# ksadov/FREUD

Hardware: AMD Instinct MI355X
Metric: SAE train activations/sec (d=384 dict 8x) (higher is better)
Workload: dtype bf16; 1 GPU; Whisper-tiny d=384 dict 8x (n=3072) L1 SAE train step, M=65536 rows/GPU/step, RAdam+cosine, x bfloat16 resident in HBM (BASELINE configs[1]); rows_per_gpu=65536, d_model=384, n_dict=3072, parallelism=dp1, dp=none

## Files before the change

### freud_amd/csrc/engine.hip

```cpp
#include <hip/hip_runtime.h>
#include <math.h>
#include <stdarg.h>
#include <stdio.h>
#include <string.h>

#include <algorithm>
#include <utility>
#include <vector>

#include "../../include/freud_sae.h"
#include "l1_kernels.h"
#include "gemm256.h"
#include "gemm256s.h"
#include "gemm256_fp8.h"
#include "l1_fp8.h"
#include "dp_kernels.h"
#include "p2p_exchange.h"
#include <rccl/rccl.h>
#include <mutex>
#include <unistd.h>

static thread_local bool g_force_gemm128 = false;
static thread_local bool g_no_stream = false;
static thread_local int g_device = 0;
// ... 115 lines not shown
  unsigned char *x8 = nullptr, *c8 = nullptr, *W8 = nullptr, *W8t = nullptr;
  float *scal8 = nullptr, *x8_part = nullptr;
  bool use_fused_fwd = false;
  int fwd_variant = 2;
  bf16_t *xb = nullptr, *c = nullptr, *dxh = nullptr, *dpre = nullptr;
  bf16_t *dxhT = nullptr, *xT = nullptr;
  float *slab = nullptr, *db_part = nullptr, *l1_part = nullptr, *sq_part = nullptr, *scal = nullptr;
  double* gn_part = nullptr;
  float* cn_part = nullptr;
  bool cn_valid = false;
  bool wb_valid = false;
  float* cnorm = nullptr;
  bool wn_pending = false, wn_fwd_seen = false;
  sae_grad_ready_fn grad_ready = nullptr;
  void* grad_ready_user = nullptr;
  int dw_chunk_rows = 0;
  int dw_chunk_splits = 1;
  int dw_col_chunks = 1;
  int dw_col_splits = 1;
  float* cnt_part = nullptr;
  int gn_blocks = 0;
  bool step_fused_call = false;
  bool gn_valid = false;
  bool metrics_fresh = false;
  const bf16_t* xb_cur = nullptr;
  unsigned int* masked = nullptr;
  int dw_splits = 1;
  int dw_tail_tiles = 0, dw_tail_pieces = 0;
  float* dw_tail = nullptr;
  int bwd_splits = 1;
  int bwd_range_splits = 1;
  bool use_fused_bwd = false;
  bool topk = false;
  int k = 0, k_aux_cap = 0;
  int64_t rows_per_file = 0;
  double dead_threshold = 1e300;
  bf16_t *We_b = nullptr, *Wd_b = nullptr, *xs = nullptr, *pre = nullptr, *dense = nullptr, *aux_dense = nullptr;
  bf16_t *de_b = nullptr, *dh_b = nullptr;
  float *e = nullptr, *dh = nullptr, *e2_part = nullptr, *a2_part = nullptr, *dbd_part = nullptr, *ds_part = nullptr, *tkf = nullptr;
  int *top_idx = nullptr, *aux_idx = nullptr, *tk = nullptr;
  bf16_t *top_vals = nullptr, *aux_vals = nullptr, *multi_vals = nullptr;
  unsigned short* tile_max = nullptr;
  unsigned char* sel_flag = nullptr;
  bool dense_valid = false;
  bool multi_dense_valid = false;
  float* be_r = nullptr;
// ... 289 lines not shown
  return SAE_OK;
}

extern "C" void sae_destroy(sae_ctx* c) {
  if (!c) return;
  (void)hipSetDevice(c->cfg.device_id);
  void* ptrs[] = {c->P,    c->Mom,     c->Var,     c->G,       c->Wb,   c->Wt,      c->xb,    c->c, c->dxh, c->dxhT, c->xT,
                  c->dpre, c->slab,    c->db_part, c->l1_part, c->sq_part, c->scal, c->gn_part, c->masked, c->cn_part, c->cnt_part,
                  c->We_b, c->Wd_b, c->xs, c->pre, c->dense, c->aux_dense, c->de_b, c->dh_b, c->e, c->dh, c->e2_part,
                  c->a2_part, c->dbd_part, c->ds_part, c->tkf, c->top_idx, c->aux_idx, c->tk, c->tv_part, c->nfsf, c->dead, c->dbe_fx,
                  c->multi_dense, c->multi_idx, c->em, c->dm_b, c->m2_part, c->x8, c->c8, c->W8, c->W8t, c->scal8, c->x8_part, c->dxh8,
                  c->stats, c->stats_part, c->Gb, c->top_vals, c->aux_vals, c->multi_vals, c->tile_max, c->sel_flag, c->csc_counts, c->csc_block_off, c->csc_total, c->csc_start, c->csc_item_start,
                  c->csc_item_latent, c->csc_entries, c->csc_part, c->csc_pbe, c->tkd, c->dead_cols, c->vec_rank, c->vec_bits, c->Wdd_b,
                  c->aux_dbe_part, c->be_r, c->cnorm, c->dw_tail, c->csc_multi, c->fs_slab};
  for (void* p : ptrs)
    if (p) (void)hipFree(p);
  if (c->dead_hint) (void)hipHostFree(c->dead_hint);
  for (int i = 0; i < c->p2p_nopened; ++i) (void)hipIpcCloseMemHandle(c->p2p_opened[i]);
  if (c->sig) (void)hipFree(c->sig);
  if (c->p2p_status) (void)hipFree(c->p2p_status);
  if (c->p2p_status_host) (void)hipHostFree(c->p2p_status_host);
  if (c->col_stage) (void)hipFree(c->col_stage);
  if (c->bal_map) (void)hipFree(c->bal_map);
  for (void* p : {(void*)c->e32_x, (void*)c->e32_pre, (void*)c->e32_sel, (void*)c->e32_xhat, (void*)c->e32_part, (void*)c->e32_colmax})
    if (p) (void)hipFree(p);
  if (c->comm) (void)ncclCommDestroy(c->comm);
  if (c->comm_stream) (void)hipStreamDestroy(c->comm_stream);
  for (hipEvent_t e : {c->ev_x, c->ev_stats, c->ev_done})
    if (e) (void)hipEventDestroy(e);
  for (hipEvent_t e : c->ev_range)
    if (e) (void)hipEventDestroy(e);
  if (c->ev_init)
    for (auto& r : c->ev)
      for (int i = 0; i < EV_RING; ++i) {
        if (r.beg[i]) (void)hipEventDestroy(r.beg[i]);
        if (r.end[i]) (void)hipEventDestroy(r.end[i]);
      }
  delete c;
}

extern "C" int sae_create(const sae_config* cfg, sae_ctx** out) {
  if (!cfg || !out) return fail(SAE_ERR_INVALID, "null argument");
  *out = nullptr;
  if (cfg->variant != SAE_VARIANT_L1 && cfg->variant != SAE_VARIANT_TOPK)
    return fail(SAE_ERR_INVALID, "Invalid autoencoder variant: %d, must be 'l1' or 'topk'", cfg->variant);
  if (cfg->variant == SAE_VARIANT_TOPK && (cfg->k <= 0 || cfg->k > cfg->n_dict || cfg->k > 1024))
// ... 159 lines not shown
  ALLOC(c->cnorm, (int64_t)c->n_p * 4);
  if (c->dw_tail_tiles > 0 || (c->d_p >= 1024 && c->d_p % 256 == 0 && c->n_p % 256 == 0)) ALLOC(c->dw_tail, (int64_t)256 * 65536 * 4);
  ALLOC(c->masked, 2048 * 4);
  ALLOC(c->cnt_part, (Mp / 128 + 1) * 4);
  c->stats_cap = DP_STATS_HEAD;
  if (!c->stats) ALLOC(c->stats, c->stats_cap * 8);
  ALLOC(c->stats_part, 1024 * 4);
  if (c->fp8) {
    ALLOC(c->x8, Mp * c->d_p);
    ALLOC(c->c8, Mp * c->n_p);
    ALLOC(c->W8, c->nW);
    ALLOC(c->W8t, c->nW);
    ALLOC(c->scal8, S8_COUNT * 4);
    ALLOC(c->x8_part, 2 * 1024 * 4);
    if (c->fp8_bwd) ALLOC(c->dxh8, Mp * c->d_p);
  }
#undef ALLOC
  {
    int rc_init = [&]() -> int {
      HIP_TRY(hipMemset(c->P, 0, c->nparams * 4));
      HIP_TRY(hipMemset(c->Mom, 0, c->nparams * 4));
      HIP_TRY(hipMemset(c->Var, 0, c->nparams * 4));
      HIP_TRY(hipMemset(c->G, 0, (c->nparams + SAE_NUM_METRICS) * 4));
      int rc_ev = create_events(c);
      if (rc_ev) return rc_ev;
      HIP_TRY(hipDeviceSynchronize());
      return SAE_OK;
    }();
    if (rc_init) {
      sae_destroy(c);
      return rc_init;
    }
  }
  *out = c;
  return SAE_OK;
}

static int copy2d(void* dst, size_t dpitch, const void* src, size_t spitch, size_t width, size_t height, int to_internal,
                  int is_device) {
  hipMemcpyKind kind = is_device ? hipMemcpyDeviceToDevice : (to_internal ? hipMemcpyHostToDevice : hipMemcpyDeviceToHost);
  HIP_TRY(hipMemcpy2D(dst, dpitch, src, spitch, width, height, kind));
  return SAE_OK;
}

static int xfer_flat(sae_ctx* c, float* internal, float* w_ext, float* b_ext, int to_internal, int is_device) {
  int rc;
// ... 910 lines not shown
    return SAE_OK;
  }
  rc = launch_encoder<T>(c, enc_gemm_args(c, c->xb_cur, Mp), M, s);
  if (rc) return rc;
  {
    GemmArgs g{};
    g.A0 = c->c; g.B0 = c->Wb; g.lda = n_p; g.ldb = n_p;
    g.nbm = (int)(Mp / 128); g.nbn = d_p / 128; g.ktiles0 = g.ktiles = n_p / 64; g.splits = 1;
    g.group_m = 4;
    EpiDec<T> e{};
    e.x = x; e.dxh = c->dxh; e.scal = c->scal; e.sq_part = c->sq_part; e.M = M; e.d = d; e.d_p = d_p; e.nbn = g.nbn;
    e.vec_all = (M == Mp && d == d_p && d % 4 == 0 && (reinterpret_cast<uintptr_t>(x) % (4 * sizeof(T))) == 0) ? 1 : 0;
    ev_begin(c, KID_DEC_FWD, s);
    rc = launch_gemm<OP_ROW, OP_ROW>(g, e, s);
    ev_end(c, KID_DEC_FWD, s);
    if (rc) return rc;
  }
  if (need_backward && c->dxhT) {
    hipLaunchKernelGGL(transpose_bf16_kernel, dim3((unsigned)(Mp / 64), d_p / 64), dim3(256), 0, s, c->dxh, c->dxhT, Mp, d_p);
    hipLaunchKernelGGL(transpose_bf16_kernel, dim3((unsigned)(Mp / 64), d_p / 64), dim3(256), 0, s, c->xb_cur, c->xT, Mp, d_p);
    HIP_TRY(hipGetLastError());
  }
  return SAE_OK;
}

template <typename T>
static int fwd_bwd_impl(sae_ctx* c, const T* x, int64_t M, hipStream_t s, bool backward) {
  const int d = c->d, d_p = c->d_p, n_p = c->n_p;
  const int64_t Mp = round_up(M, c->row_pad);
  const float alpha = (float)c->cfg.recon_alpha;
  const double* gs = (backward && c->dp_world > 0) ? c->stats : nullptr;
  ev_begin(c, KID_STEP_TOTAL, s);
  int rc = forward_impl<T>(c, x, M, Mp, s, backward);
  if (rc) return rc;
  const bool fold_finalize = c->use_fused_fwd && c->use_fused_bwd && backward && gs == nullptr && c->bwd_ranges == 1 &&
                             c->cfg.debug_flags != 78;
  if (c->use_fused_fwd && !fold_finalize) {
    StatsPush push{};
    if (gs && inline_stats(c)) {
      for (int r = 0; r < c->dp_world; ++r) push.inbox[r] = c->p2p_sig[r] + P2P_SIG_WORDS;
      push.rank = c->p2p_rank; push.world = c->dp_world; push.epoch = ++c->p2p_epoch_push;
      push.timeout_ticks = c->p2p_timeout_ticks; push.status = c->p2p_status; push.status_host = c->p2p_status_hostdev; push.gstats_out = c->stats;
    } else if (gs && c->dist) {
      HIP_TRY(hipStreamWaitEvent(s, c->ev_stats, 0));
    }
    if (push.world > 0) ev_begin(c, KID_STATS_XCHG, s);
// ... 161 lines not shown
        rc = launch_dw(g, e, r0);
        if (rc) return rc;
        if (direct && g.tail_tiles > 0)
          hipLaunchKernelGGL(reduce_tail_kernel, dim3(g.tail_tiles, 16), dim3(256), 0, s, c->dw_tail, c->G, n_p, d_p / 256, n_p / 256,
                             g.tail_tiles, g.tail_pieces);
        if (chunked) {
          const int64_t off4 = (int64_t)r0 * n_p / 4, n4 = (int64_t)rows * n_p / 4;
          hipLaunchKernelGGL(reduce_slabs_kernel, dim3((unsigned)((n4 + 255) / 256)), dim3(256), 0, s, c->slab + 4 * off4,
                             c->G + 4 * off4, n4, c->nW / 4, splits);
          notify_grads(c, 4 * off4, 4 * n4, s);
        }
      }
      if (!col_chunked) {
        ev_end(c, KID_DW, s);
        dw_chunked_any = chunked;
        dw_chunked = chunked || direct;
      }
    }
    ev_begin(c, KID_REDUCE, s);
    if (c->use_fused_bwd && c->bwd_ranges > 1) {
      c->gn_blocks = 256 * c->bwd_ranges;
      c->gn_valid = true;
    } else if (c->use_fused_bwd) {
      const int64_t nW4 = c->nW / 4, n4 = c->nparams / 4;
      const int blocks = grid_for(n4, 1024);
      LossFinalize fin{};
      if (fold_finalize) {
        fin.l1_part = c->l1_part; fin.sq_part = c->sq_part; fin.cnt_part = c->cnt_part; fin.n_parts = (int)(Mp / 128);
        fin.scal = c->scal; fin.metrics = c->G + c->nparams; fin.M = M; fin.d = d; fin.alpha = alpha;
      }
      hipLaunchKernelGGL(reduce_grads_kernel, dim3(blocks), dim3(256), 0, s, c->slab, nW4, splits, c->db_part, db_rows, n_p,
                         c->G, nW4, n4, c->gn_part,
                         (c->dist && c->dp_world > 0 && c->payload == SAE_DTYPE_BF16) ? c->Gb : (bf16_t*)nullptr, fin,
                         (c->bwd_ranges == 1 && c->bal_m > 0 && (int)(Mp / BF_BM) >= 64) ? c->bal_m : 0);
      c->gn_blocks = blocks;
      c->gn_valid = true;
    } else {
      const int64_t n4 = c->nW / 4;
      if (!dw_chunked)
        hipLaunchKernelGGL(reduce_slabs_kernel, dim3((unsigned)((n4 + 255) / 256)), dim3(256), 0, s, c->slab, c->G, n4, n4,
                           splits);
      hipLaunchKernelGGL(reduce_db_kernel, dim3(n_p / 32), dim3(256), 0, s, c->db_part, c->G + c->nW, db_rows, n_p);
      c->gn_valid = false;
    }
    ev_end(c, KID_REDUCE, s);
  }
  if (!c->use_fused_fwd)
    hipLaunchKernelGGL(finalize_losses_kernel, dim3(1), dim3(1024), 0, s, c->l1_part, (int)((Mp / 128) * (n_p / 128)),
                       c->sq_part, (int)((Mp / 128) * (d_p / 128)), c->scal, c->G + c->nparams, M, d, alpha,
                       (const float*)nullptr, 0, gs, StatsPush{});
  if (backward) {
    const int64_t total = c->nparams + SAE_NUM_METRICS;
    if (c->use_fused_bwd && c->dist && c->dp_world > 0) {
      const int nr = c->bwd_ranges, cols = n_p / nr;
      fused_exchange(c, nr - 1, nr, (nr - 1) * cols, cols, true, s);
    } else if (dw_chunked_any) notify_grads(c, c->nW, total - c->nW, s);
    else notify_grads(c, 0, total, s);
  }
  ev_end(c, KID_STEP_TOTAL, s);
// ... 544 lines not shown
  a.grad_scale = (float)grad_scale;
  a.clip_thresh = (float)c->cfg.clip_thresh;
  a.weight_decay = (float)c->cfg.weight_decay;
  a.beta1 = (float)b1;
  a.beta2 = (float)b2;
  a.eps = (float)c->cfg.eps;
  a.one_minus_beta1 = (float)(1.0 - b1);
  a.one_minus_beta2 = (float)(1.0 - b2);
  a.bc1 = (float)bc1;
  a.bc2_sqrt = (float)sqrt(bc2);
  a.step_size = (float)(lr / bc1);
  a.is_radam = c->cfg.optimizer == SAE_OPT_RADAM;
  a.scale_metrics = c->metrics_fresh ? 1 : 0;
  c->metrics_fresh = false;
  if (a.is_radam) {
    const double rho_inf = 2.0 / (1.0 - b2) - 1.0;
    const double rho_t = rho_inf - 2.0 * t * pow(b2, t) / bc2;
    a.rectify = rho_t > 5.0;
    a.rect = a.rectify ? (float)sqrt((rho_t - 4) * (rho_t - 2) * rho_inf / ((rho_inf - 4) * (rho_inf - 2) * rho_t)) : 0.f;
  }
  ev_begin(c, KID_OPT, s);
  const int64_t n4 = c->nparams / 4;
  int gblocks = grid_for(n4, 1024);
  if (c->grads_in_bf16) {
    hipLaunchKernelGGL(gnorm_from_bf16_kernel, dim3(gblocks), dim3(256), 0, s, c->Gb, c->G, n4, a.grad_scale, c->gn_part);
    c->grads_in_bf16 = false;
  } else if (c->gn_valid && grad_scale == 1.0 && c->step_fused_call) {
    gblocks = c->gn_blocks;
  } else {
    hipLaunchKernelGGL(gnorm_partial_kernel, dim3(gblocks), dim3(256), 0, s, c->G, n4, a.grad_scale, c->gn_part);
  }
  c->gn_valid = false;
  const int oblocks = grid_for(n4, 2048);
  if (!c->topk && !c->fp8 && c->d_p <= 384 && c->cfg.debug_flags != 79 && c->cfg.debug_flags != 80) {
    const int norm_on_load = (c->wn_pending && c->wn_fwd_seen) ? 1 : 0;
    hipLaunchKernelGGL(optimizer_l1_cols_kernel, dim3(c->n_p / OPTC_COLS + c->n_p / 128), dim3(OPTC_THREADS), optc_lds_bytes(c->d_p), s, c->P,
                       c->Mom, c->Var, c->G, c->d_p, c->n_p, c->gn_part, gblocks, a, c->G + c->nparams, c->cnorm, norm_on_load, c->Wb,
                       c->Wt);
    c->wn_pending = true;
    c->wn_fwd_seen = false;
    c->cn_valid = false;
  } else if (!c->topk && c->cfg.debug_flags != 79) {
    settle_weights(c, s);
    hipLaunchKernelGGL(optimizer_l1_kernel, dim3(c->n_p / 128, c->d_p / 32 + 1), dim3(256), 0, s, c->P, c->Mom, c->Var, c->G, c->d_p,
                       c->n_p, c->gn_part, gblocks, a, c->G + c->nparams, c->cn_part);
    c->cn_valid = true;
// ... 7 lines not shown
    hipLaunchKernelGGL(optimizer_kernel, dim3(oblocks), dim3(256), 0, s, c->P, c->Mom, c->Var, c->G, n4, c->gn_part, gblocks,
                       a, c->G + c->nparams, cast);
    c->cn_valid = false;
    c->wb_valid = c->topk;
  }
  if (c->topk)
    hipLaunchKernelGGL(nfsf_update_kernel, dim3((c->n + 255) / 256), dim3(256), 0, s, c->nfsf, c->G + c->nparams + SAE_NUM_METRICS,
                       c->n, (long long)(c->last_M * (grad_scale > 0 ? (long long)llround(1.0 / grad_scale) : 1)),
                       c->dp_world > 0 ? c->stats : (const double*)nullptr);
  ev_end(c, KID_OPT, s);
  HIP_TRY(hipGetLastError());
  return SAE_OK;
}

extern "C" int sae_set_topk_options(sae_ctx* c, double dead_feature_threshold, int64_t rows_per_file) {
  if (!c) return fail(SAE_ERR_INVALID, "null argument");
  if (!c->topk) return fail(SAE_ERR_STATE, "not a topk context");
  c->dead_threshold = dead_feature_threshold;
  c->rows_per_file = rows_per_file;
  return SAE_OK;
}

extern "C" int sae_step(sae_ctx* c, const void* x, int64_t M, int x_dtype, double lr, void* stream) {
  int rc = sae_forward_backward(c, x, M, x_dtype, stream);
  if (rc) return rc;
  c->step_fused_call = c->dp_world == 0 || c->gn_from_exchange;
  rc = sae_optimizer_step(c, lr, 1.0, stream);
  c->step_fused_call = false;
  return rc;
}

extern "C" int sae_read_metrics(sae_ctx* c, float out[SAE_NUM_METRICS], void* stream) {
  if (!c || !out) return fail(SAE_ERR_INVALID, "null argument");
  if (int rc = no_forward_left(c)) return rc;
  USE_DEVICE(c);
  HIP_TRY(hipMemcpyAsync(out, c->G + c->nparams, SAE_NUM_METRICS * 4, hipMemcpyDeviceToHost, (hipStream_t)stream));
  HIP_TRY(hipStreamSynchronize((hipStream_t)stream));
  return SAE_OK;
}

static int ensure_dense(sae_ctx* c) {
  if (!c->topk || c->dense_valid || c->last_M <= 0) return SAE_OK;
  HIP_TRY(hipDeviceSynchronize());
  hipLaunchKernelGGL(topk_densify_kernel, dim3((unsigned)c->last_M_p), dim3(256), 0, (hipStream_t)0, c->top_vals, c->top_idx, c->k,
                     c->dense, c->n_p);
  HIP_TRY(hipGetLastError());
  HIP_TRY(hipDeviceSynchronize());
  c->dense_valid = true;
  return SAE_OK;
}

extern "C" int sae_debug_read(sae_ctx* c, int which, float* out, int64_t cap) {
  if (!c || !out) return fail(SAE_ERR_INVALID, "null argument");
  USE_DEVICE(c);
  HIP_TRY(hipDeviceSynchronize());
  if (which == 0) {
    int rc_d = ensure_dense(c);
    if (rc_d) return rc_d;
  }
  const int64_t M = c->last_M;
// ... 54 lines not shown
  if (which == 12) {
    const int64_t rows = cap / 8 < 4096 ? cap / 8 : 4096;
    std::vector<unsigned long long> tmp((size_t)rows * 8);
    HIP_TRY(hipMemcpyFromSymbol(tmp.data(), HIP_SYMBOL(tsel_stamp_buf), tmp.size() * 8, 0, hipMemcpyDeviceToHost));
    for (int64_t i = 0; i < rows * 8; ++i) out[i] = (float)tmp[(size_t)i];
    return SAE_OK;
  }
#endif
  if (which == 11) {
    if (!c->topk || !c->aux_dense) return fail(SAE_ERR_INVALID, "no AuxK buffers");
    const int64_t rows = cap / 8 < c->last_M ? cap / 8 : c->last_M;
    std::vector<unsigned long long> tmp((size_t)rows * 8);
    HIP_TRY(hipMemcpy2D(tmp.data(), 64, reinterpret_cast<const char*>(c->aux_dense) + (size_t)c->n_p * 2 - 64, (size_t)c->n_p * 2, 64, (size_t)rows,
                        hipMemcpyDeviceToHost));
    for (int64_t i = 0; i < rows * 8; ++i) out[i] = (float)tmp[(size_t)i];
    return SAE_OK;
  }
  if (which == 5) {
    const int64_t nq = (c->last_M / FF_BM) * 4 * 8;
    if (cap < nq) return fail(SAE_ERR_INVALID, "capacity too small");
    std::vector<unsigned long long> tmp((size_t)nq);
    HIP_TRY(hipMemcpy(tmp.data(), c->dpre, tmp.size() * 8, hipMemcpyDeviceToHost));
    for (int64_t i = 0; i < nq; ++i) out[i] = (float)tmp[(size_t)i];
    return SAE_OK;
  }
  if (which == 2 && c->topk) {
    const int64_t nd = (int64_t)c->n * c->d;
    if (cap < 2 * nd + c->n + c->d) return fail(SAE_ERR_INVALID, "capacity too small");
    float* const ext[4] = {out, out + nd, out + nd + c->n, out + 2 * nd + c->n};
    return xfer_flat_topk(c, c->G, ext, 0, 0);
  }
  if (which == 3 && c->topk) {
    if (cap < M * c->k) return fail(SAE_ERR_INVALID, "capacity too small");
    std::vector<int> tmp((size_t)M * c->k);
    HIP_TRY(hipMemcpy(tmp.data(), c->top_idx, tmp.size() * 4, hipMemcpyDeviceToHost));
    for (size_t i = 0; i < tmp.size(); ++i) out[i] = (float)tmp[i];
    return SAE_OK;
  }
  if (which == 2) {
    if (cap < (int64_t)c->d * c->n + c->n) return fail(SAE_ERR_INVALID, "capacity too small");
    int rc = xfer_flat(c, c->G, out, out + (int64_t)c->d * c->n, 0, 0);
    return rc;
  }
  return fail(SAE_ERR_INVALID, "unknown debug tensor %d", which);
}

// ... 417 lines not shown
```

### freud_amd/csrc/l1_kernels.h

```cpp
#pragma once
#include "gemm.h"

__device__ __forceinline__ float colnorm_tree8(const float (*red)[128], int col) {
  return ((red[0][col] + red[1][col]) + (red[2][col] + red[3][col])) + ((red[4][col] + red[5][col]) + (red[6][col] + red[7][col]));
}

__global__ __launch_bounds__(256) void colnorm_partial_kernel(const float* __restrict__ W, float* __restrict__ part,
                                                               int n_p) {
  __shared__ float red[8][128];
  const int t = threadIdx.x, tx = t & 31, ty = t >> 5;
  const int col = blockIdx.x * 128 + 4 * tx, r0 = blockIdx.y * 32;
  f32x4 ss = {0.f, 0.f, 0.f, 0.f};
#pragma unroll
  for (int i = 0; i < 4; ++i) {
    const f32x4 v = *reinterpret_cast<const f32x4*>(W + (int64_t)(r0 + ty + 8 * i) * n_p + col);
#pragma unroll
    for (int q = 0; q < 4; ++q) ss[q] = __builtin_fmaf(v[q], v[q], ss[q]);
  }
#pragma unroll
  for (int q = 0; q < 4; ++q) red[ty][4 * tx + q] = ss[q];
  __syncthreads();
  if (t < 128) part[(int64_t)blockIdx.y * n_p + blockIdx.x * 128 + t] = colnorm_tree8(red, t);
}

// ... 395 lines not shown

__global__ __launch_bounds__(256) void reduce_slabs_kernel(const float* __restrict__ slab, float* __restrict__ grad,
                                                            int64_t n4, int64_t stride4, int splits) {
  const int64_t i = (int64_t)blockIdx.x * 256 + threadIdx.x;
  if (i >= n4) return;
  const f32x4* s = reinterpret_cast<const f32x4*>(slab);
  f32x4 a = s[i];
  for (int k = 1; k < splits; ++k) a += s[i + k * stride4];
  reinterpret_cast<f32x4*>(grad)[i] = a;
}

struct LossFinalize {
  const float *l1_part, *sq_part, *cnt_part;
  int n_parts;
  float *scal, *metrics;
  int64_t M;
  int d;
  float alpha;
};

__device__ __forceinline__ void finalize_losses_block256(const LossFinalize& f) {
  __shared__ double redf[4][4];
  double a = 0, b = 0, c = 0, m = 0;
  for (int i = threadIdx.x; i < f.n_parts; i += 256) {
    a += (double)f.l1_part[i];
    b += (double)f.sq_part[2 * i];
    c += (double)f.sq_part[2 * i + 1];
    m += (double)f.cnt_part[i];
  }
  a = wave_sum_d(a); b = wave_sum_d(b); c = wave_sum_d(c); m = wave_sum_d(m);
  if ((threadIdx.x & 63) == 0) {
    const int w = threadIdx.x >> 6;
    redf[0][w] = a; redf[1][w] = b; redf[2][w] = c; redf[3][w] = m;
  }
  __syncthreads();
  if (threadIdx.x == 0) {
    const double l1 = (redf[0][0] + redf[0][1]) + (redf[0][2] + redf[0][3]), sq = (redf[1][0] + redf[1][1]) + (redf[1][2] + redf[1][3]);
    const double pl = (redf[2][0] + redf[2][1]) + (redf[2][2] + redf[2][3]), masked = (redf[3][0] + redf[3][1]) + (redf[3][2] + redf[3][3]);
    const double local = (double)f.M * f.d - masked;
    f.scal[0] = (float)local;
    f.scal[1] = f.alpha / (float)local;
    f.scal[2] = 1.0f / (float)f.M;
    f.scal[3] = (float)local;
    const double count = (double)f.scal[0];
    f.metrics[0] = (float)((double)f.alpha * (sq / count));
    f.metrics[1] = (float)(l1 / (double)f.M);
    f.metrics[2] = (float)(pl / ((double)f.M * f.d));
    f.metrics[3] = 0.f;
    f.metrics[4] = f.scal[0];
    f.metrics[5] = f.metrics[6] = f.metrics[7] = 0.f;
  }
}

__global__ __launch_bounds__(256) void reduce_grads_kernel(const float* __restrict__ slab, int64_t stride4, int splits,
                                                            const float* __restrict__ db_part, int db_rows, int n_p,
                                                            float* __restrict__ grad, int64_t nW4, int64_t n4,
                                                            double* __restrict__ gn_part, bf16_t* __restrict__ grad_bf16,
                                                            LossFinalize fin, int bal_m) {
  __shared__ double red[4];
  if (fin.cnt_part && blockIdx.x == gridDim.x - 1) finalize_losses_block256(fin);
  double ss = 0;
  const int n4p = n_p / 4;
  auto add_pieces = [](f32x4 a, const f32x4* p, int64_t stride, int cnt) -> f32x4 {
    int k = 1;
    for (; k + 7 < cnt; k += 8) {
      f32x4 v[8];
#pragma unroll
      for (int u = 0; u < 8; ++u) v[u] = p[(k + u) * stride];
#pragma unroll
      for (int u = 0; u < 8; ++u) a += v[u];
    }
    if (k + 3 < cnt) {
      f32x4 v[4];
#pragma unroll
      for (int u = 0; u < 4; ++u) v[u] = p[(k + u) * stride];
#pragma unroll
      for (int u = 0; u < 4; ++u) a += v[u];
      k += 4;
    }
    if (k + 1 < cnt) {
      const f32x4 v0 = p[k * stride], v1 = p[(k + 1) * stride];
      a += v0;
      a += v1;
      k += 2;
    }
    if (k < cnt) a += p[k * stride];
    return a;
  };
  for (int64_t i = (int64_t)blockIdx.x * 256 + threadIdx.x; i < n4; i += (int64_t)gridDim.x * 256) {
    f32x4 a;
    if (i < nW4) {
      const f32x4* s = reinterpret_cast<const f32x4*>(slab);
      const int cnt = bal_m > 0 ? bal_pieces((int)(i % n4p) >> 5, bal_m) : splits;
      a = add_pieces(s[i], s + i, stride4, cnt);
    } else {
      const int64_t j4 = i - nW4;
      const f32x4* s = reinterpret_cast<const f32x4*>(db_part);
      const int cnt = bal_m > 0 ? bal_pieces((int)j4 >> 5, bal_m) : db_rows;
      a = add_pieces(s[j4], s + j4, (int64_t)n4p, cnt);
    }
    reinterpret_cast<f32x4*>(grad)[i] = a;
    if (grad_bf16) reinterpret_cast<bf16x4*>(grad_bf16)[i] = bf16x4{(bf16_t)a[0], (bf16_t)a[1], (bf16_t)a[2], (bf16_t)a[3]};
    ss += (double)(a[0] * a[0]) + (double)(a[1] * a[1]) + (double)(a[2] * a[2]) + (double)(a[3] * a[3]);
  }
  ss = wave_sum_d(ss);
  if ((threadIdx.x & 63) == 0) red[threadIdx.x >> 6] = ss;
  __syncthreads();
  if (threadIdx.x == 0) gn_part[blockIdx.x] = red[0] + red[1] + red[2] + red[3];
}

__global__ __launch_bounds__(256) void gnorm_from_bf16_kernel(const bf16_t* __restrict__ gb, float* __restrict__ grad, int64_t n4,
// ... 314 lines not shown
    if (t < 32) update4((int64_t)d_p * n_p + blockIdx.x * 128 + 4 * t);
    return;
  }
  const int col = blockIdx.x * 128 + 4 * tx, r0 = blockIdx.y * 32;
  f32x4 ss = {0.f, 0.f, 0.f, 0.f};
#pragma unroll
  for (int i = 0; i < 4; ++i) {
    const f32x4 pv = update4((int64_t)(r0 + ty + 8 * i) * n_p + col);
#pragma unroll
    for (int q = 0; q < 4; ++q) ss[q] = __builtin_fmaf(pv[q], pv[q], ss[q]);
  }
#pragma unroll
  for (int q = 0; q < 4; ++q) red[ty][4 * tx + q] = ss[q];
  __syncthreads();
  if (t < 128) cn_part[(int64_t)blockIdx.y * n_p + blockIdx.x * 128 + t] = colnorm_tree8(red, t);
}

constexpr int OPTC_COLS = 16, OPTC_THREADS = 512, OPTC_MAX_PASS = 3;
constexpr int OPTC_TPR = OPTC_COLS / 4;
constexpr int OPTC_ROWS = OPTC_THREADS / OPTC_TPR;
static_assert(OPTC_ROWS == 128, "rows ty + 128 i: d_p is a multiple of 128");
__host__ __device__ constexpr int optc_lds_bytes(int d_p) { return (d_p * OPTC_COLS + (d_p / 32) * 8 * OPTC_COLS + OPTC_COLS) * 4; }

__global__ __launch_bounds__(OPTC_THREADS) void optimizer_l1_cols_kernel(float* __restrict__ p, float* __restrict__ m, float* __restrict__ v,
                                                                          const float* __restrict__ grad, int d_p, int n_p,
                                                                          const double* __restrict__ gn_part, int n_part, OptArgs a,
                                                                          float* __restrict__ metrics, float* __restrict__ cnorm,
                                                                          int norm_on_load, bf16_t* __restrict__ Wb, bf16_t* __restrict__ Wt) {
  extern __shared__ __attribute__((aligned(16))) float optc_smem[];
  __shared__ double redd[OPTC_THREADS / 64];
  const int t = threadIdx.x, nslab = d_p / 32, npass = d_p / 128;
  const int ncb = n_p / OPTC_COLS;
  const bool bias_block = (int)blockIdx.x >= ncb;
  float* pn = optc_smem;
  float* red = pn + d_p * OPTC_COLS;
  float* den = red + nslab * 8 * OPTC_COLS;
  const int cblk = bias_block ? 0 : ((int)blockIdx.x & 7) * (ncb >> 3) + ((int)blockIdx.x >> 3);
  const int col0 = cblk * OPTC_COLS;
  const int tx = t % OPTC_TPR, ty = t / OPTC_TPR;
  f32x4 dn = {1.f, 1.f, 1.f, 1.f};
  f32x4 g[OPTC_MAX_PASS], pv[OPTC_MAX_PASS], mv[OPTC_MAX_PASS], vv[OPTC_MAX_PASS];
  if (!bias_block) {
    if (norm_on_load) dn = *reinterpret_cast<const f32x4*>(cnorm + col0 + 4 * tx);
#pragma unroll
    for (int i = 0; i < OPTC_MAX_PASS; ++i)
      if (i < npass) {
        const int64_t o = (int64_t)(128 * i + ty) * n_p + col0 + 4 * tx;
        g[i] = *reinterpret_cast<const f32x4*>(grad + o);
        pv[i] = *reinterpret_cast<f32x4*>(p + o);
        mv[i] = *reinterpret_cast<f32x4*>(m + o);
        vv[i] = *reinterpret_cast<f32x4*>(v + o);
      }
  }
  float coef;
  {
    double sg = 0;
    for (int i = t; i < n_part; i += OPTC_THREADS) sg += gn_part[i];
    sg = wave_sum_d(sg);
    if ((t & 63) == 0) redd[t >> 6] = sg;
    __syncthreads();
    double tot = 0;
#pragma unroll
    for (int w = 0; w < OPTC_THREADS / 64; ++w) tot += redd[w];
    const float total = sqrtf((float)tot);
    if (blockIdx.x == 0 && t == 0) {
      metrics[3] = total;
      if (a.scale_metrics && a.grad_scale != 1.0f) {
        metrics[0] *= a.grad_scale;
        metrics[1] *= a.grad_scale;
        metrics[2] *= a.grad_scale;
        metrics[5] *= a.grad_scale;
      }
    }
    coef = fminf(a.clip_thresh / (total + 1e-6f), 1.0f);
  }
  if (bias_block) {
    if (t < 32) {
      const int64_t o = (int64_t)d_p * n_p + ((int)blockIdx.x - ncb) * 128 + 4 * t;
      const f32x4 gb = *reinterpret_cast<const f32x4*>(grad + o);
      f32x4 pb = *reinterpret_cast<f32x4*>(p + o), mb = *reinterpret_cast<f32x4*>(m + o), vb = *reinterpret_cast<f32x4*>(v + o);
      adam_update4(gb, pb, mb, vb, a, coef);
      *reinterpret_cast<f32x4*>(p + o) = pb;
      *reinterpret_cast<f32x4*>(m + o) = mb;
      *reinterpret_cast<f32x4*>(v + o) = vb;
    }
    return;
  }
#pragma unroll
  for (int i = 0; i < OPTC_MAX_PASS; ++i)
    if (i < npass) {
      const int row = 128 * i + ty;
      const int64_t o = (int64_t)row * n_p + col0 + 4 * tx;
      if (norm_on_load) {
#pragma unroll
        for (int q = 0; q < 4; ++q) pv[i][q] = pv[i][q] / dn[q];
      }
      adam_update4(g[i], pv[i], mv[i], vv[i], a, coef);
      *reinterpret_cast<f32x4*>(p + o) = pv[i];
      *reinterpret_cast<f32x4*>(m + o) = mv[i];
      *reinterpret_cast<f32x4*>(v + o) = vv[i];
      *reinterpret_cast<f32x4*>(pn + row * OPTC_COLS + 4 * tx) = pv[i];
    }
  __syncthreads();
  {
    const int cc = t % OPTC_COLS;
    for (int pr = t / OPTC_COLS; pr < nslab * 8; pr += OPTC_THREADS / OPTC_COLS) {
      const int i = pr >> 3, y8 = pr & 7;
      float ss = 0.f;
#pragma unroll
      for (int k = 0; k < 4; ++k) {
        const float w = pn[(32 * i + y8 + 8 * k) * OPTC_COLS + cc];
        ss = __builtin_fmaf(w, w, ss);
      }
      red[pr * OPTC_COLS + cc] = ss;
    }
  }
  __syncthreads();
  if (t < OPTC_COLS) {
// ... 8 lines not shown
  }
  __syncthreads();
  {
    const f32x4 dn = *reinterpret_cast<const f32x4*>(den + 4 * tx);
#pragma unroll
    for (int i = 0; i < OPTC_MAX_PASS; ++i)
      if (i < npass) {
        const int row = 128 * i + ty;
        const f32x4 w = *reinterpret_cast<const f32x4*>(pn + row * OPTC_COLS + 4 * tx);
        *reinterpret_cast<bf16x4*>(Wb + (int64_t)row * n_p + col0 + 4 * tx) =
            bf16x4{(bf16_t)(w[0] / dn[0]), (bf16_t)(w[1] / dn[1]), (bf16_t)(w[2] / dn[2]), (bf16_t)(w[3] / dn[3])};
      }
    const int cc = t % OPTC_COLS;
    const float dc = den[cc];
    for (int pc = t / OPTC_COLS; pc < d_p / 8; pc += OPTC_THREADS / OPTC_COLS) {
      bf16x8 o;
#pragma unroll
      for (int e = 0; e < 8; ++e) o[e] = (bf16_t)(pn[(8 * pc + e) * OPTC_COLS + cc] / dc);
      *reinterpret_cast<bf16x8*>(Wt + (int64_t)(col0 + cc) * d_p + 8 * pc) = o;
    }
  }
}

__global__ __launch_bounds__(256) void normalize_inplace_kernel(float* __restrict__ W, const float* __restrict__ cnorm, int64_t n4, int n_p) {
  for (int64_t i = (int64_t)blockIdx.x * 256 + threadIdx.x; i < n4; i += (int64_t)gridDim.x * 256) {
    const int col = (int)((4 * i) % n_p);
    f32x4 w = reinterpret_cast<f32x4*>(W)[i];
    const f32x4 dn = *reinterpret_cast<const f32x4*>(cnorm + col);
#pragma unroll
    for (int q = 0; q < 4; ++q) w[q] = w[q] / dn[q];
    reinterpret_cast<f32x4*>(W)[i] = w;
  }
}

template <typename T>
__global__ __launch_bounds__(256) void pad_latent_kernel(const T* __restrict__ src, int64_t ld, int64_t M, int n,
                                                          bf16_t* __restrict__ dst, int64_t M_p, int n_p) {
  const int64_t total = M_p * (int64_t)n_p;
  for (int64_t i = (int64_t)blockIdx.x * 256 + threadIdx.x; i < total; i += (int64_t)gridDim.x * 256) {
    const int64_t r = i / n_p;
    const int c = (int)(i - r * n_p);
    dst[i] = (r < M && c < n) ? (bf16_t)(float)src[r * ld + c] : (bf16_t)0.f;
  }
}

struct EpiStoreF32 {
// ... 16 lines not shown
```

Baseline: 122.4 million activations/s.

## Fuse gradient reduction, clip and L1 optimizer update into one cooperative kernel

When the step runs single-GPU with the fused backward, it defers the gradient-reduction launch and instead launches a cooperative kernel. That kernel sums the split gradient pieces, computes per-block norm partials, and synchronizes all workgroups through a global atomic counter with a timeout. It then applies clipping and the column-normalized Adam update while the reduced gradients are still in registers. This removes a separate reduce launch and a re-read of the gradient buffer, at the cost of a grid-wide spin barrier that requires all blocks to be co-resident, with fallback and error reporting if the barrier times out.

```diff
diff --git a/freud_amd/csrc/engine.hip b/freud_amd/csrc/engine.hip
--- a/freud_amd/csrc/engine.hip
+++ b/freud_amd/csrc/engine.hip
@@ -161,6 +161,13 @@
   int gn_blocks = 0;
   bool step_fused_call = false;
   bool gn_valid = false;
+  int num_cus = 0;
+  bool tail_armed = false, tail_pending = false, tail_refused = false;
+  struct { int splits, db_rows, bal_m; LossFinalize fin; } tail_args = {};
+  unsigned long long* tail_sync = nullptr;
+  unsigned long long tail_epoch = 0;
+  unsigned int* tail_status_host = nullptr;
+  unsigned int* tail_status_hostdev = nullptr;
   bool metrics_fresh = false;
   const bf16_t* xb_cur = nullptr;
   unsigned int* masked = nullptr;
@@ -496,6 +503,8 @@
   if (c->p2p_status_host) (void)hipHostFree(c->p2p_status_host);
   if (c->col_stage) (void)hipFree(c->col_stage);
   if (c->bal_map) (void)hipFree(c->bal_map);
+  if (c->tail_sync) (void)hipFree(c->tail_sync);
+  if (c->tail_status_host) (void)hipHostFree(c->tail_status_host);
   for (void* p : {(void*)c->e32_x, (void*)c->e32_pre, (void*)c->e32_sel, (void*)c->e32_xhat, (void*)c->e32_part, (void*)c->e32_colmax})
     if (p) (void)hipFree(p);
   if (c->comm) (void)ncclCommDestroy(c->comm);
@@ -701,6 +710,18 @@
       HIP_TRY(hipMemset(c->Mom, 0, c->nparams * 4));
       HIP_TRY(hipMemset(c->Var, 0, c->nparams * 4));
       HIP_TRY(hipMemset(c->G, 0, (c->nparams + SAE_NUM_METRICS) * 4));
+      if (c->use_fused_bwd && c->use_fused_fwd) {
+        HIP_TRY(hipDeviceGetAttribute(&c->num_cus, hipDeviceAttributeMultiprocessorCount, c->cfg.device_id));
+        HIP_TRY(hipMalloc((void**)&c->tail_sync, 64));
+        HIP_TRY(hipMemset(c->tail_sync, 0, 64));
+        if (hipHostMalloc((void**)&c->tail_status_host, 64, hipHostMallocMapped) == hipSuccess) {
+          memset(c->tail_status_host, 0, 64);
+          if (hipHostGetDevicePointer((void**)&c->tail_status_hostdev, c->tail_status_host, 0) != hipSuccess) c->tail_status_hostdev = nullptr;
+        } else {
+          (void)hipGetLastError();
+          c->tail_status_host = nullptr;
+        }
+      }
       int rc_ev = create_events(c);
       if (rc_ev) return rc_ev;
       HIP_TRY(hipDeviceSynchronize());
@@ -1657,6 +1678,23 @@
     HIP_TRY(hipGetLastError());
   }
   return SAE_OK;
+}
+
+static void launch_reduce_grads(sae_ctx* c, int splits, int db_rows, int bal_m, const LossFinalize& fin, hipStream_t s) {
+  const int64_t nW4 = c->nW / 4, n4 = c->nparams / 4;
+  const int blocks = grid_for(n4, 1024);
+  hipLaunchKernelGGL(reduce_grads_kernel, dim3(blocks), dim3(256), 0, s, c->slab, nW4, splits, c->db_part, db_rows, c->n_p,
+                     c->G, nW4, n4, c->gn_part,
+                     (c->dist && c->dp_world > 0 && c->payload == SAE_DTYPE_BF16) ? c->Gb : (bf16_t*)nullptr, fin, bal_m);
+  c->gn_blocks = blocks;
+  c->gn_valid = true;
+}
+
+static unsigned long long tail_timeout_ticks(const sae_ctx* c) { return c->p2p_timeout_ticks < 200000000ull ? c->p2p_timeout_ticks : 200000000ull; }
+static int tail_grid(const sae_ctx* c) { return c->n_p / OPTC_COLS + c->n_p / 128; }
+static bool tail_fusable(const sae_ctx* c) {
+  return c->tail_sync != nullptr && !c->tail_refused && c->dp_world == 0 && !c->dist && c->use_fused_bwd && c->bwd_ranges == 1 && !c->topk &&
+         !c->fp8 && c->d_p <= 384 && c->cfg.debug_flags == 0 && c->grad_ready == nullptr && tail_grid(c) <= c->num_cus;
 }
 
 template <typename T>
@@ -1864,19 +1902,19 @@
       c->gn_blocks = 256 * c->bwd_ranges;
       c->gn_valid = true;
     } else if (c->use_fused_bwd) {
-      const int64_t nW4 = c->nW / 4, n4 = c->nparams / 4;
-      const int blocks = grid_for(n4, 1024);
       LossFinalize fin{};
       if (fold_finalize) {
         fin.l1_part = c->l1_part; fin.sq_part = c->sq_part; fin.cnt_part = c->cnt_part; fin.n_parts = (int)(Mp / 128);
         fin.scal = c->scal; fin.metrics = c->G + c->nparams; fin.M = M; fin.d = d; fin.alpha = alpha;
       }
-      hipLaunchKernelGGL(reduce_grads_kernel, dim3(blocks), dim3(256), 0, s, c->slab, nW4, splits, c->db_part, db_rows, n_p,
-                         c->G, nW4, n4, c->gn_part,
-                         (c->dist && c->dp_world > 0 && c->payload == SAE_DTYPE_BF16) ? c->Gb : (bf16_t*)nullptr, fin,
-                         (c->bwd_ranges == 1 && c->bal_m > 0 && (int)(Mp / BF_BM) >= 64) ? c->bal_m : 0);
-      c->gn_blocks = blocks;
-      c->gn_valid = true;
+      const int bal_m = (c->bwd_ranges == 1 && c->bal_m > 0 && (int)(Mp / BF_BM) >= 64) ? c->bal_m : 0;
+      if (c->tail_armed && fold_finalize && tail_fusable(c)) {
+        c->tail_args.splits = splits; c->tail_args.db_rows = db_rows; c->tail_args.bal_m = bal_m; c->tail_args.fin = fin;
+        c->tail_pending = true;
+        c->gn_valid = false;
+      } else {
+        launch_reduce_grads(c, splits, db_rows, bal_m, fin, s);
+      }
     } else {
       const int64_t n4 = c->nW / 4;
       if (!dw_chunked)
@@ -2467,6 +2505,37 @@
   ev_begin(c, KID_OPT, s);
   const int64_t n4 = c->nparams / 4;
   int gblocks = grid_for(n4, 1024);
+  if (c->tail_pending) {
+    c->tail_pending = false;
+    const int norm_on_load = (c->wn_pending && c->wn_fwd_seen) ? 1 : 0;
+    const int grid = tail_grid(c);
+    TailSync sync{};
+    sync.counter = c->tail_sync; sync.epoch = c->tail_epoch + 1; sync.timeout_ticks = tail_timeout_ticks(c);
+    sync.status = reinterpret_cast<unsigned int*>(c->tail_sync + 1); sync.status_host = c->tail_status_hostdev;
+    float *P = c->P, *Mo = c->Mom, *Va = c->Var, *G = c->G, *metrics = c->G + c->nparams, *cnorm = c->cnorm;
+    const float *slab = c->slab, *db_part = c->db_part;
+    int d_p = c->d_p, n_p = c->n_p, splits = c->tail_args.splits, db_rows = c->tail_args.db_rows, bal_m = c->tail_args.bal_m, nol = norm_on_load;
+    int64_t stride4 = c->nW / 4;
+    double* gn = c->gn_part;
+    bf16_t *Wb = c->Wb, *Wt = c->Wt;
+    LossFinalize fin = c->tail_args.fin;
+    void* args[] = {&P, &Mo, &Va, &G, &d_p, &n_p, &slab, &stride4, &splits, &db_part, &db_rows, &bal_m, &gn, &a, &metrics, &cnorm, &nol,
+                    &Wb, &Wt, &fin, &sync};
+    const hipError_t e = hipLaunchCooperativeKernel(reinterpret_cast<const void*>(&reduce_clip_update_l1_cols_kernel), dim3(grid),
+                                                    dim3(OPTC_THREADS), args, (unsigned)optc_lds_bytes(c->d_p), s);
+    if (e == hipSuccess) {
+      c->tail_epoch += 1;
+      c->wn_pending = true;
+      c->wn_fwd_seen = false;
+      c->cn_valid = false;
+      ev_end(c, KID_OPT, s);
+      HIP_TRY(hipGetLastError());
+      return SAE_OK;
+    }
+    (void)hipGetLastError();
+    c->tail_refused = true;
+    launch_reduce_grads(c, splits, db_rows, bal_m, fin, s);
+  }
   if (c->grads_in_bf16) {
     hipLaunchKernelGGL(gnorm_from_bf16_kernel, dim3(gblocks), dim3(256), 0, s, c->Gb, c->G, n4, a.grad_scale, c->gn_part);
     c->grads_in_bf16 = false;
@@ -2520,8 +2589,16 @@
 }
 
 extern "C" int sae_step(sae_ctx* c, const void* x, int64_t M, int x_dtype, double lr, void* stream) {
+  if (c && c->tail_status_host && *(volatile unsigned int*)c->tail_status_host)
+    return fail(SAE_ERR_STATE, "the fused update gave up waiting for its workgroups (%.1f s): the optimizer state of this context is incomplete",
+                tail_timeout_ticks(c) / 1e8);
+  if (c) c->tail_armed = true;
   int rc = sae_forward_backward(c, x, M, x_dtype, stream);
-  if (rc) return rc;
+  if (c) c->tail_armed = false;
+  if (rc) {
+    if (c) c->tail_pending = false;
+    return rc;
+  }
   c->step_fused_call = c->dp_world == 0 || c->gn_from_exchange;
   rc = sae_optimizer_step(c, lr, 1.0, stream);
   c->step_fused_call = false;
@@ -2534,6 +2611,9 @@
   USE_DEVICE(c);
   HIP_TRY(hipMemcpyAsync(out, c->G + c->nparams, SAE_NUM_METRICS * 4, hipMemcpyDeviceToHost, (hipStream_t)stream));
   HIP_TRY(hipStreamSynchronize((hipStream_t)stream));
+  if (c->tail_status_host && *(volatile unsigned int*)c->tail_status_host)
+    return fail(SAE_ERR_STATE, "the fused update gave up waiting for its workgroups (%.1f s): the optimizer state of this context is incomplete",
+                tail_timeout_ticks(c) / 1e8);
   return SAE_OK;
 }
 
@@ -2634,6 +2714,24 @@
     std::vector<unsigned long long> tmp((size_t)nq);
     HIP_TRY(hipMemcpy(tmp.data(), c->dpre, tmp.size() * 8, hipMemcpyDeviceToHost));
     for (int64_t i = 0; i < nq; ++i) out[i] = (float)tmp[(size_t)i];
+    return SAE_OK;
+  }
+  if (which == 14 && !c->topk) {
+    if (cap < 2 * c->nW) return fail(SAE_ERR_INVALID, "capacity too small");
+    std::vector<uint16_t> tmp((size_t)c->nW);
+    for (int h = 0; h < 2; ++h) {
+      HIP_TRY(hipMemcpy(tmp.data(), h == 0 ? c->Wb : c->Wt, tmp.size() * 2, hipMemcpyDeviceToHost));
+      for (int64_t i = 0; i < c->nW; ++i) {
+        const uint32_t u = (uint32_t)tmp[(size_t)i] << 16;
+        memcpy(out + h * c->nW + i, &u, 4);
+      }
+    }
+    return SAE_OK;
+  }
+  if (which == 15) {
+    if (cap < 4) return fail(SAE_ERR_INVALID, "capacity too small");
+    out[0] = (float)c->tail_epoch; out[1] = c->tail_refused ? 1.f : 0.f; out[2] = (float)c->num_cus;
+    out[3] = c->topk ? 0.f : (float)tail_grid(c);
     return SAE_OK;
   }
   if (which == 2 && c->topk) {
diff --git a/freud_amd/csrc/l1_kernels.h b/freud_amd/csrc/l1_kernels.h
--- a/freud_amd/csrc/l1_kernels.h
+++ b/freud_amd/csrc/l1_kernels.h
@@ -441,14 +441,14 @@
 __device__ __forceinline__ void finalize_losses_block256(const LossFinalize& f) {
   __shared__ double redf[4][4];
   double a = 0, b = 0, c = 0, m = 0;
-  for (int i = threadIdx.x; i < f.n_parts; i += 256) {
+  for (int i = threadIdx.x; i < f.n_parts && threadIdx.x < 256; i += 256) {
     a += (double)f.l1_part[i];
     b += (double)f.sq_part[2 * i];
     c += (double)f.sq_part[2 * i + 1];
     m += (double)f.cnt_part[i];
   }
   a = wave_sum_d(a); b = wave_sum_d(b); c = wave_sum_d(c); m = wave_sum_d(m);
-  if ((threadIdx.x & 63) == 0) {
+  if ((threadIdx.x & 63) == 0 && threadIdx.x < 256) {
     const int w = threadIdx.x >> 6;
     redf[0][w] = a; redf[1][w] = b; redf[2][w] = c; redf[3][w] = m;
   }
@@ -471,6 +471,33 @@
   }
 }
 
+__device__ __forceinline__ f32x4 add_pieces(f32x4 a, const f32x4* p, int64_t stride, int cnt) {
+  int k = 1;
+  for (; k + 7 < cnt; k += 8) {
+    f32x4 v[8];
+#pragma unroll
+    for (int u = 0; u < 8; ++u) v[u] = p[(k + u) * stride];
+#pragma unroll
+    for (int u = 0; u < 8; ++u) a += v[u];
+  }
+  if (k + 3 < cnt) {
+    f32x4 v[4];
+#pragma unroll
+    for (int u = 0; u < 4; ++u) v[u] = p[(k + u) * stride];
+#pragma unroll
+    for (int u = 0; u < 4; ++u) a += v[u];
+    k += 4;
+  }
+  if (k + 1 < cnt) {
+    const f32x4 v0 = p[k * stride], v1 = p[(k + 1) * stride];
+    a += v0;
+    a += v1;
+    k += 2;
+  }
+  if (k < cnt) a += p[k * stride];
+  return a;
+}
+
 __global__ __launch_bounds__(256) void reduce_grads_kernel(const float* __restrict__ slab, int64_t stride4, int splits,
                                                             const float* __restrict__ db_part, int db_rows, int n_p,
                                                             float* __restrict__ grad, int64_t nW4, int64_t n4,
@@ -480,32 +507,6 @@
   if (fin.cnt_part && blockIdx.x == gridDim.x - 1) finalize_losses_block256(fin);
   double ss = 0;
   const int n4p = n_p / 4;
-  auto add_pieces = [](f32x4 a, const f32x4* p, int64_t stride, int cnt) -> f32x4 {
-    int k = 1;
-    for (; k + 7 < cnt; k += 8) {
-      f32x4 v[8];
-#pragma unroll
-      for (int u = 0; u < 8; ++u) v[u] = p[(k + u) * stride];
-#pragma unroll
-      for (int u = 0; u < 8; ++u) a += v[u];
-    }
-    if (k + 3 < cnt) {
-      f32x4 v[4];
-#pragma unroll
-      for (int u = 0; u < 4; ++u) v[u] = p[(k + u) * stride];
-#pragma unroll
-      for (int u = 0; u < 4; ++u) a += v[u];
-      k += 4;
-    }
-    if (k + 1 < cnt) {
-      const f32x4 v0 = p[k * stride], v1 = p[(k + 1) * stride];
-      a += v0;
-      a += v1;
-      k += 2;
-    }
-    if (k < cnt) a += p[k * stride];
-    return a;
-  };
   for (int64_t i = (int64_t)blockIdx.x * 256 + threadIdx.x; i < n4; i += (int64_t)gridDim.x * 256) {
     f32x4 a;
     if (i < nW4) {
@@ -866,70 +867,81 @@
 static_assert(OPTC_ROWS == 128, "rows ty + 128 i: d_p is a multiple of 128");
 __host__ __device__ constexpr int optc_lds_bytes(int d_p) { return (d_p * OPTC_COLS + (d_p / 32) * 8 * OPTC_COLS + OPTC_COLS) * 4; }
 
-__global__ __launch_bounds__(OPTC_THREADS) void optimizer_l1_cols_kernel(float* __restrict__ p, float* __restrict__ m, float* __restrict__ v,
-                                                                          const float* __restrict__ grad, int d_p, int n_p,
-                                                                          const double* __restrict__ gn_part, int n_part, OptArgs a,
-                                                                          float* __restrict__ metrics, float* __restrict__ cnorm,
-                                                                          int norm_on_load, bf16_t* __restrict__ Wb, bf16_t* __restrict__ Wt) {
-  extern __shared__ __attribute__((aligned(16))) float optc_smem[];
-  __shared__ double redd[OPTC_THREADS / 64];
-  const int t = threadIdx.x, nslab = d_p / 32, npass = d_p / 128;
-  const int ncb = n_p / OPTC_COLS;
-  const bool bias_block = (int)blockIdx.x >= ncb;
-  float* pn = optc_smem;
-  float* red = pn + d_p * OPTC_COLS;
-  float* den = red + nslab * 8 * OPTC_COLS;
-  const int cblk = bias_block ? 0 : ((int)blockIdx.x & 7) * (ncb >> 3) + ((int)blockIdx.x >> 3);
-  const int col0 = cblk * OPTC_COLS;
-  const int tx = t % OPTC_TPR, ty = t / OPTC_TPR;
-  f32x4 dn = {1.f, 1.f, 1.f, 1.f};
-  f32x4 g[OPTC_MAX_PASS], pv[OPTC_MAX_PASS], mv[OPTC_MAX_PASS], vv[OPTC_MAX_PASS];
-  if (!bias_block) {
-    if (norm_on_load) dn = *reinterpret_cast<const f32x4*>(cnorm + col0 + 4 * tx);
-#pragma unroll
-    for (int i = 0; i < OPTC_MAX_PASS; ++i)
-      if (i < npass) {
-        const int64_t o = (int64_t)(128 * i + ty) * n_p + col0 + 4 * tx;
-        g[i] = *reinterpret_cast<const f32x4*>(grad + o);
-        pv[i] = *reinterpret_cast<f32x4*>(p + o);
-        mv[i] = *reinterpret_cast<f32x4*>(m + o);
-        vv[i] = *reinterpret_cast<f32x4*>(v + o);
-      }
-  }
-  float coef;
-  {
-    double sg = 0;
-    for (int i = t; i < n_part; i += OPTC_THREADS) sg += gn_part[i];
-    sg = wave_sum_d(sg);
-    if ((t & 63) == 0) redd[t >> 6] = sg;
-    __syncthreads();
-    double tot = 0;
-#pragma unroll
-    for (int w = 0; w < OPTC_THREADS / 64; ++w) tot += redd[w];
-    const float total = sqrtf((float)tot);
-    if (blockIdx.x == 0 && t == 0) {
-      metrics[3] = total;
-      if (a.scale_metrics && a.grad_scale != 1.0f) {
-        metrics[0] *= a.grad_scale;
-        metrics[1] *= a.grad_scale;
-        metrics[2] *= a.grad_scale;
-        metrics[5] *= a.grad_scale;
-      }
-    }
-    coef = fminf(a.clip_thresh / (total + 1e-6f), 1.0f);
-  }
-  if (bias_block) {
-    if (t < 32) {
-      const int64_t o = (int64_t)d_p * n_p + ((int)blockIdx.x - ncb) * 128 + 4 * t;
-      const f32x4 gb = *reinterpret_cast<const f32x4*>(grad + o);
-      f32x4 pb = *reinterpret_cast<f32x4*>(p + o), mb = *reinterpret_cast<f32x4*>(m + o), vb = *reinterpret_cast<f32x4*>(v + o);
-      adam_update4(gb, pb, mb, vb, a, coef);
-      *reinterpret_cast<f32x4*>(p + o) = pb;
-      *reinterpret_cast<f32x4*>(m + o) = mb;
-      *reinterpret_cast<f32x4*>(v + o) = vb;
-    }
-    return;
-  }
+struct OptcBlock {
+  int t, tx, ty, nslab, npass, ncb, col0;
+  bool bias_block;
+  float *pn, *red, *den;
+};
+
+__device__ __forceinline__ OptcBlock optc_block(float* smem, int d_p, int n_p) {
+  OptcBlock b;
+  b.t = threadIdx.x; b.nslab = d_p / 32; b.npass = d_p / 128;
+  b.ncb = n_p / OPTC_COLS;
+  b.bias_block = (int)blockIdx.x >= b.ncb;
+  b.pn = smem;
+  b.red = b.pn + d_p * OPTC_COLS;
+  b.den = b.red + b.nslab * 8 * OPTC_COLS;
+  const int cblk = b.bias_block ? 0 : ((int)blockIdx.x & 7) * (b.ncb >> 3) + ((int)blockIdx.x >> 3);
+  b.col0 = cblk * OPTC_COLS;
+  b.tx = b.t % OPTC_TPR; b.ty = b.t / OPTC_TPR;
+  return b;
+}
+
+template <bool AGENT>
+__device__ __forceinline__ float optc_clip_coef(const double* __restrict__ gn_part, int n_part, const OptArgs& a,
+                                                float* __restrict__ metrics, double* redd, bool publish) {
+  const int t = threadIdx.x;
+  double sg = 0;
+  for (int i = t; i < n_part; i += OPTC_THREADS)
+    sg += AGENT ? __hip_atomic_load(gn_part + i, __ATOMIC_RELAXED, __HIP_MEMORY_SCOPE_AGENT) : gn_part[i];
+  sg = wave_sum_d(sg);
+  if ((t & 63) == 0) redd[t >> 6] = sg;
+  __syncthreads();
+  double tot = 0;
+#pragma unroll
+  for (int w = 0; w < OPTC_THREADS / 64; ++w) tot += redd[w];
+  const float total = sqrtf((float)tot);
+  if (publish && t == 0) {
+    metrics[3] = total;
+    if (a.scale_metrics && a.grad_scale != 1.0f) {
+      metrics[0] *= a.grad_scale;
+      metrics[1] *= a.grad_scale;
+      metrics[2] *= a.grad_scale;
+      metrics[5] *= a.grad_scale;
+    }
+  }
+  return fminf(a.clip_thresh / (total + 1e-6f), 1.0f);
+}
+
+__device__ __forceinline__ void optc_bias_update(int64_t o, const f32x4 gb, float* __restrict__ p, float* __restrict__ m,
+                                                 float* __restrict__ v, const OptArgs& a, float coef) {
+  f32x4 pb = *reinterpret_cast<f32x4*>(p + o), mb = *reinterpret_cast<f32x4*>(m + o), vb = *reinterpret_cast<f32x4*>(v + o);
+  adam_update4(gb, pb, mb, vb, a, coef);
+  *reinterpret_cast<f32x4*>(p + o) = pb;
+  *reinterpret_cast<f32x4*>(m + o) = mb;
+  *reinterpret_cast<f32x4*>(v + o) = vb;
+}
+
+__device__ __forceinline__ void optc_load_state(const OptcBlock& b, const float* __restrict__ p, const float* __restrict__ m,
+                                                const float* __restrict__ v, const float* __restrict__ cnorm, int norm_on_load,
+                                                int n_p, f32x4& dn, f32x4* pv, f32x4* mv, f32x4* vv) {
+  if (norm_on_load) dn = *reinterpret_cast<const f32x4*>(cnorm + b.col0 + 4 * b.tx);
+#pragma unroll
+  for (int i = 0; i < OPTC_MAX_PASS; ++i)
+    if (i < b.npass) {
+      const int64_t o = (int64_t)(128 * i + b.ty) * n_p + b.col0 + 4 * b.tx;
+      pv[i] = *reinterpret_cast<const f32x4*>(p + o);
+      mv[i] = *reinterpret_cast<const f32x4*>(m + o);
+      vv[i] = *reinterpret_cast<const f32x4*>(v + o);
+    }
+}
+
+__device__ __forceinline__ void optc_update_cols(const OptcBlock& b, const f32x4* g, f32x4* pv, f32x4* mv, f32x4* vv, const f32x4 dn_old,
+                                                 float* __restrict__ p, float* __restrict__ m, float* __restrict__ v, int d_p, int n_p,
+                                                 const OptArgs& a, float coef, float* __restrict__ cnorm, int norm_on_load,
+                                                 bf16_t* __restrict__ Wb, bf16_t* __restrict__ Wt) {
+  const int t = b.t, tx = b.tx, ty = b.ty, col0 = b.col0, nslab = b.nslab, npass = b.npass;
+  float *pn = b.pn, *red = b.red, *den = b.den;
 #pragma unroll
   for (int i = 0; i < OPTC_MAX_PASS; ++i)
     if (i < npass) {
@@ -937,7 +949,7 @@
       const int64_t o = (int64_t)row * n_p + col0 + 4 * tx;
       if (norm_on_load) {
 #pragma unroll
-        for (int q = 0; q < 4; ++q) pv[i][q] = pv[i][q] / dn[q];
+        for (int q = 0; q < 4; ++q) pv[i][q] = pv[i][q] / dn_old[q];
       }
       adam_update4(g[i], pv[i], mv[i], vv[i], a, coef);
       *reinterpret_cast<f32x4*>(p + o) = pv[i];
@@ -992,6 +1004,122 @@
   }
 }
 
+__global__ __launch_bounds__(OPTC_THREADS) void optimizer_l1_cols_kernel(float* __restrict__ p, float* __restrict__ m, float* __restrict__ v,
+                                                                          const float* __restrict__ grad, int d_p, int n_p,
+                                                                          const double* __restrict__ gn_part, int n_part, OptArgs a,
+                                                                          float* __restrict__ metrics, float* __restrict__ cnorm,
+                                                                          int norm_on_load, bf16_t* __restrict__ Wb, bf16_t* __restrict__ Wt) {
+  extern __shared__ __attribute__((aligned(16))) float optc_smem[];
+  __shared__ double redd[OPTC_THREADS / 64];
+  const OptcBlock b = optc_block(optc_smem, d_p, n_p);
+  f32x4 dn = {1.f, 1.f, 1.f, 1.f};
+  f32x4 g[OPTC_MAX_PASS], pv[OPTC_MAX_PASS], mv[OPTC_MAX_PASS], vv[OPTC_MAX_PASS];
+  if (!b.bias_block) {
+#pragma unroll
+    for (int i = 0; i < OPTC_MAX_PASS; ++i)
+      if (i < b.npass) g[i] = *reinterpret_cast<const f32x4*>(grad + (int64_t)(128 * i + b.ty) * n_p + b.col0 + 4 * b.tx);
+    optc_load_state(b, p, m, v, cnorm, norm_on_load, n_p, dn, pv, mv, vv);
+  }
+  const float coef = optc_clip_coef<false>(gn_part, n_part, a, metrics, redd, blockIdx.x == 0);
+  if (b.bias_block) {
+    if (b.t < 32) {
+      const int64_t o = (int64_t)d_p * n_p + ((int)blockIdx.x - b.ncb) * 128 + 4 * b.t;
+      optc_bias_update(o, *reinterpret_cast<const f32x4*>(grad + o), p, m, v, a, coef);
+    }
+    return;
+  }
+  optc_update_cols(b, g, pv, mv, vv, dn, p, m, v, d_p, n_p, a, coef, cnorm, norm_on_load, Wb, Wt);
+}
+
+struct TailSync {
+  unsigned long long* counter;
+  unsigned long long epoch;
+  unsigned long long timeout_ticks;
+  unsigned int* status;
+  unsigned int* status_host;
+};
+
+__global__ __launch_bounds__(OPTC_THREADS) void reduce_clip_update_l1_cols_kernel(
+    float* __restrict__ p, float* __restrict__ m, float* __restrict__ v, float* __restrict__ grad, int d_p, int n_p,
+    const float* __restrict__ slab, int64_t stride4, int splits, const float* __restrict__ db_part, int db_rows, int bal_m,
+    double* gn_part, OptArgs a, float* metrics, float* __restrict__ cnorm, int norm_on_load, bf16_t* __restrict__ Wb,
+    bf16_t* __restrict__ Wt, LossFinalize fin, TailSync sync) {
+  extern __shared__ __attribute__((aligned(16))) float optc_smem[];
+  __shared__ double redd[OPTC_THREADS / 64];
+  __shared__ int gave_up;
+  const OptcBlock b = optc_block(optc_smem, d_p, n_p);
+  const int t = b.t, n4p = n_p / 4;
+  f32x4 dn = {1.f, 1.f, 1.f, 1.f};
+  f32x4 g[OPTC_MAX_PASS], pv[OPTC_MAX_PASS], mv[OPTC_MAX_PASS], vv[OPTC_MAX_PASS];
+  const int64_t ob = (int64_t)d_p * n_p + ((int)blockIdx.x - b.ncb) * 128 + 4 * t;
+  double ss = 0;
+  if (!b.bias_block) {
+    optc_load_state(b, p, m, v, cnorm, norm_on_load, n_p, dn, pv, mv, vv);
+    const int cnt = bal_m > 0 ? bal_pieces(b.col0 >> 7, bal_m) : splits;
+    const f32x4* s = reinterpret_cast<const f32x4*>(slab);
+#pragma unroll
+    for (int i = 0; i < OPTC_MAX_PASS; ++i)
+      if (i < b.npass) {
+        const int64_t o4 = ((int64_t)(128 * i + b.ty) * n_p + b.col0) / 4 + b.tx;
+        g[i] = add_pieces(s[o4], s + o4, stride4, cnt);
+        ss += (double)(g[i][0] * g[i][0]) + (double)(g[i][1] * g[i][1]) + (double)(g[i][2] * g[i][2]) + (double)(g[i][3] * g[i][3]);
+      }
+  } else if (t < 32) {
+    const int64_t j4 = (int64_t)((int)blockIdx.x - b.ncb) * 32 + t;
+    const f32x4* s = reinterpret_cast<const f32x4*>(db_part);
+    const int cnt = bal_m > 0 ? bal_pieces((int)j4 >> 5, bal_m) : db_rows;
+    g[0] = add_pieces(s[j4], s + j4, (int64_t)n4p, cnt);
+    ss = (double)(g[0][0] * g[0][0]) + (double)(g[0][1] * g[0][1]) + (double)(g[0][2] * g[0][2]) + (double)(g[0][3] * g[0][3]);
+  }
+  ss = wave_sum_d(ss);
+  if ((t & 63) == 0) redd[t >> 6] = ss;
+  if (t == 0) gave_up = 0;
+  __syncthreads();
+  if (t == 0) {
+    double tot = 0;
+#pragma unroll
+    for (int w = 0; w < OPTC_THREADS / 64; ++w) tot += redd[w];
+    __hip_atomic_store(gn_part + blockIdx.x, tot, __ATOMIC_RELAXED, __HIP_MEMORY_SCOPE_AGENT);
+    __threadfence();
+    asm volatile("s_waitcnt vmcnt(0)" ::: "memory");
+    atomicAdd(sync.counter, 1ull);
+  }
+  if (!b.bias_block) {
+#pragma unroll
+    for (int i = 0; i < OPTC_MAX_PASS; ++i)
+      if (i < b.npass) *reinterpret_cast<f32x4*>(grad + (int64_t)(128 * i + b.ty) * n_p + b.col0 + 4 * b.tx) = g[i];
+  } else if (t < 32) {
+    *reinterpret_cast<f32x4*>(grad + ob) = g[0];
+  }
+  if (t == 0) {
+    const unsigned long long target = sync.epoch * gridDim.x, t0 = __builtin_amdgcn_s_memrealtime();
+    while (__hip_atomic_load(sync.counter, __ATOMIC_RELAXED, __HIP_MEMORY_SCOPE_AGENT) < target) {
+      __builtin_amdgcn_s_sleep(2);
+      if (__builtin_amdgcn_s_memrealtime() - t0 > sync.timeout_ticks) {
+        gave_up = 1;
+        atomicOr(sync.status, 1u);
+        if (sync.status_host) __hip_atomic_store(sync.status_host, 1u, __ATOMIC_RELAXED, __HIP_MEMORY_SCOPE_SYSTEM);
+        break;
+      }
+    }
+    __threadfence();
+    asm volatile("s_waitcnt vmcnt(0)" ::: "memory");
+  }
+  __syncthreads();
+  if (gave_up) return;
+  const bool last = blockIdx.x == gridDim.x - 1;
+  if (fin.cnt_part && last) {
+    finalize_losses_block256(fin);
+    __syncthreads();
+  }
+  const float coef = optc_clip_coef<true>(gn_part, (int)gridDim.x, a, metrics, redd, last);
+  if (b.bias_block) {
+    if (t < 32) optc_bias_update(ob, g[0], p, m, v, a, coef);
+    return;
+  }
+  optc_update_cols(b, g, pv, mv, vv, dn, p, m, v, d_p, n_p, a, coef, cnorm, norm_on_load, Wb, Wt);
+}
+
 __global__ __launch_bounds__(256) void normalize_inplace_kernel(float* __restrict__ W, const float* __restrict__ cnorm, int64_t n4, int n_p) {
   for (int64_t i = (int64_t)blockIdx.x * 256 + threadIdx.x; i < n4; i += (int64_t)gridDim.x * 256) {
     const int col = (int)((4 * i) % n_p);
```

New measurement: 118.4 million activations/s. -3.2%, worse.
